# geometryxyz/mental-poker

Measured on AMD Instinct MI355X. Metric: shuffle proofs/sec (prove+verify), higher is better.
Workload: dtype u32 limbs (256-bit Montgomery: 9x29-bit lazy base field, 8x32 scalar field); 1 GPU; pairs: 52-card deck, m=2 n=26, stark curve, shuffle_and_remask + verify_shuffle; rccl_world=1, fixed_base_window_bits=21, unit_counted=prove+verify pairs, streams=1, aggregate_keys=1, transcript_lanes=1, prover_streams=1, pipeline_depth=0, validated_once=False, full=False

## Files before the change

mental-poker_amd/csrc/engine_core.hpp:

```cpp
#pragma once
#include "engine_base.hpp"
#include "kernels_bucket.hpp"
#include "kernels_canonical.hpp"
#include "kernels_sigma.hpp"
#include "kernels_open.hpp"
#include "kernels_deal.hpp"
#include "kernels_sample.hpp"
#include "kernels_screen.hpp"
#include "serialize_host.hpp"
#include "setup_host.hpp"

namespace mp {

static const uint32_t FCHUNK = 8;
static const uint32_t VCHUNK = 64;
static const uint32_t NORM_CHUNK = 64;
static const uint32_t BUCKET_MIN = 2048;
static const uint32_t BUCKET_MIN_SMALL_BATCH = 512;

struct PhaseDev {
  DevBuf<Term> recode, tables, fterms, vterms, cterms, cterms2, cterms0;
  DevBuf<Job> fjobs, vjobs, cjobs, cjobs2, cjobs0;
  DevBuf<BJob> bjobs;
  DevBuf<Term> bterms;
  DevBuf<BTermPos> bpos;
  DevBuf<Job> wcjobs;
  DevBuf<Term> wcterms;
  DevBuf<BJob> wjobs;
  uint32_t vsplit = 1, n_wc = 0, n_w = 0;
  uint32_t n_b = 0, n_bterms = 0, b_dig_bytes = 0, b_kpad_max = 0, b_bits = 8;
  uint32_t n_recode = 0, n_tables = 0, n_f = 0, n_v = 0, n_c = 0, n_c2 = 0, n_c0 = 0, n_tslots = 0, n_dslots = 0;
  std::vector<std::pair<uint32_t, uint32_t>> normalize;
  void upload(const Phase& ph, rt::Stream s) {
    recode.upload(ph.recode, s);
    tables.upload(ph.tables, s);
    fterms.upload(ph.fterms, s);
    vterms.upload(ph.vterms, s);
    cterms.upload(ph.cterms, s);
    fjobs.upload(ph.fjobs, s);
    vjobs.upload(ph.vjobs, s);
    cjobs.upload(ph.cjobs, s);
    cterms2.upload(ph.cterms2, s);
    cjobs2.upload(ph.cjobs2, s);
    n_c2 = (uint32_t)ph.cjobs2.size();
    cterms0.upload(ph.cterms0, s);
    cjobs0.upload(ph.cjobs0, s);
    n_c0 = (uint32_t)ph.cjobs0.size();
    wcjobs.upload(ph.wcjobs, s);
    wcterms.upload(ph.wcterms, s);
    wjobs.upload(ph.wjobs, s);
    vsplit = ph.vsplit;
    n_wc = (uint32_t)ph.wcjobs.size();
    n_w = (uint32_t)ph.wjobs.size();
    bjobs.upload(ph.bjobs, s);
    bterms.upload(ph.bterms, s);
    bpos.upload(ph.bpos, s);
    n_b = (uint32_t)ph.bjobs.size();
    n_bterms = (uint32_t)ph.bterms.size();
    b_dig_bytes = ph.b_dig_bytes;
    b_kpad_max = ph.b_kpad_max;
    b_bits = ph.b_bits;
    n_recode = (uint32_t)ph.recode.size();
    n_tables = (uint32_t)ph.tables.size();
    n_f = (uint32_t)ph.fjobs.size();
    n_v = (uint32_t)ph.vjobs.size();
    n_c = (uint32_t)ph.cjobs.size();
    n_tslots = ph.n_tslots;
    n_dslots = ph.n_dslots;
// ... 262 lines not shown
    rt::stream_sync(s);
  }
  DevBuf<uint32_t> vflag;
  uint32_t* flag_word(bool vlane, rt::Stream s) {
    if (!vflag.n) vflag.alloc(2, s);
    rt::dzero(vflag.p + (vlane ? 1 : 0), 4, s);
    return vflag.p + (vlane ? 1 : 0);
  }
  bool read_flag(bool vlane) {
    uint32_t flag = 0;
    rt::d2h(&flag, vflag.p + (vlane ? 1 : 0), 4, ctx->stream);
    rt::stream_sync(ctx->stream);
    return flag != 0;
  }
  uint32_t nwin = 0;
  FbGeom fbg{8, 32, 255};
  uint32_t init_seed[8];
  DevBuf<uint8_t> io_a, io_b, io_c, io_d, io_e, io_f;
  DevBuf<int32_t> io_status;

  static bool wire_point_host(const uint8_t* p, Aff<C>& out) {
    alignas(8) uint8_t tmp[G_::PB];
    memcpy(tmp, p, G_::PB);
    return wire_to_aff<C>(tmp, out);
  }

  void build_plans(PlanSet* set, bool keyed) {
    rt::Stream s = ctx->stream;
    for (int k = 0; k < N_PLANS; ++k) {
      PlanSet& q = set[k];
      const PlanParams& pp = pprm[k];
      const uint32_t bmin = (bucket_min && k == 3) ? std::min(bucket_min, BUCKET_MIN_SMALL_BATCH) : bucket_min;
      const uint32_t pbits = bucket_bits_of(4 * N + 11 * m + 9);
      q.pplan = make_prove_plan(m, n, pp.fch, pp.vch, G_::PB, keyed, bmin, bk_windows(R::BITS, pbits), toom_cook && (k == 0 || k == 2 || k == 4), pp.vsp, pbits);
      q.vplan = make_verify_plan(m, n, pp.fch, pp.vch, G_::PB, keyed, bmin, bk_windows(R::BITS, pbits), pp.vsp, pbits);
      q.table_group = pp.grp;
      q.norm_chunk = pp.nch;
      for (int i = 0; i < 6; ++i) q.pph[i].upload(q.pplan.ph[i], s);
      q.vph.upload(q.vplan.ph, s);
      q.vmph.upload(q.vplan.mph, s);
      q.mjobs.upload(q.vplan.mjobs, s);
      q.mpairs.upload(q.vplan.mpairs, s);
      q.draws.upload(q.pplan.draws, s);
      q.lin.upload(q.pplan.lin, s);
      q.lin_src.upload(q.pplan.lin_src, s);
      q.lin_coef.upload(q.pplan.lin_coef, s);
      q.consts.upload(toom_constants(q.pplan.toom), s);
      q.pwire.upload(q.pplan.wire, s);
      q.vwire.upload(q.vplan.wire, s);
    }
  }
  void ensure_keyed() {
    if (psk_ready) return;
    build_plans(psk, true);
    const ProveLay& l = psk[0].pplan.lay;
    key_d_first = key_t_first = 0;
    for (int k = 0; k < N_PLANS; ++k)
      for (int i = 0; i < 6; ++i) {
        key_d_first = std::max(key_d_first, psk[k].pplan.ph[i].n_dslots);
        key_t_first = std::max(key_t_first, psk[k].pplan.ph[i].n_tslots);
      }
    std::vector<Term> rec, tab;
    for (uint32_t i = 0; i < N; ++i) rec.push_back(Term{l.rho + i, key_d_first + i});
    for (uint32_t w = 0; w < nwin; ++w) tab.push_back(Term{l.kw + w, key_t_first + w});
    key_recode.upload(rec, ctx->stream);
    key_tables.upload(tab, ctx->stream);
    psk_ready = true;
// ... 187 lines not shown
    if (!scratch) scratch = w.NS.p;
    if (parts & PH_TABLES) run_tables(ph, w, B, scratch);
    if (parts & PH_RECODE) run_recode(ph, w, B);
    if (parts & PH_MSM) run_msms(ph, w, B);
    if (parts & PH_NORM) run_normalize(ph, w, B, norm_only, norm_skip, scratch);
  }
#ifdef MP_EXP_QUAD_MAX
  uint32_t quad_max_lanes = MP_EXP_QUAD_MAX;
#else
  uint32_t quad_max_lanes = 65536;
#endif
  bool quad_ops(uint32_t B, uint32_t njobs) const {
    const uint64_t items = (uint64_t)B * njobs;
    if (items > 0xFFFFFFF0ull) return false;
    return group_lanes == 4 || (group_lanes == 0 && items * 4u <= quad_max_lanes);
  }
  static uint32_t quad_waves(uint32_t B, uint32_t njobs) { return (uint32_t)(((uint64_t)B * njobs + 15u) / 16u); }
  void run_combine(const CombineArgs& a, uint32_t B, uint32_t njobs) {
    if (quad_ops(B, njobs)) {
      CombineQuadArgs qa{a, B, njobs};
      MP_WAVE_RUN(k_combine_q, C, quad_waves(B, njobs), 0, qa);
    } else {
      MP_RUN(k_combine, C, B, njobs, a);
    }
  }
  void run_recode(PhaseDev& ph, Workspace& w, uint32_t B) {
    if (ph.n_recode) {
      RecodeArgs a{w.S.p, w.D.p, ph.recode.p, w.Bpad, nwin};
      MP_RUN(k_recode, C, B, ph.n_recode, a);
    }
  }
  void run_tables(PhaseDev& ph, Workspace& w, uint32_t B, uint32_t* scratch) {
    if (ph.n_tables) {
      TableArgs a{w.P.p, w.T.p, scratch, ph.tables.p, w.Bpad, ph.n_tables, cur_table_group};
      MP_RUN(k_table, C, B, (ph.n_tables + cur_table_group - 1) / cur_table_group, a);
    }
  }

  uint32_t bk_pass_eqs = 0;
  size_t bk_pass_bytes = 0;
  uint32_t bucket_slots() {
    if (!ctx->bk_slots) ctx->bk_slots = BK_WAVES_PER_CU * rt::cu_count();
    return ctx->bk_slots;
  }
  void run_bucket(Workspace& w, PhaseDev& ph, const uint32_t* S, uint32_t sstride, int16_t* D, size_t dstride, uint32_t count,
                  uint32_t link_stride, const char* too_large, const uint32_t* tile = nullptr, uint32_t tile_K = 0) {
    rt::Stream s = ctx->stream;
    const uint32_t c = ph.b_bits, bw = bk_windows(R::BITS, c);
    if ((uint64_t)count * ph.n_bterms >= ((uint64_t)1 << 32) || (uint64_t)count * ph.n_b * bw + 8ull * bucket_slots() >= ((uint64_t)1 << 32)) throw std::runtime_error(too_large);
    BRecodeArgs ra{S, D, ph.bterms.p, ph.bpos.p, sstride, bw, ph.n_bterms, dstride, c};
    MP_RUN(k_bucket_recode, C, count * ph.n_bterms, 1, ra);
    if (c >= bucket_split_bits) {
      const uint32_t NBK = bk_buckets(c), XW = XyzzWords<C>::N, gmax = bk_chunks(ph.b_kpad_max), units = bk_units(c);
      if (gmax > BK_CHUNKS_MAX) throw std::runtime_error("bucket method: more than 589 824 terms in one multi-scalar multiplication with windows of 12 bits or more");
      const size_t per_item = ((size_t)ph.b_kpad_max + (size_t)NBK * XW) * 4 + (size_t)gmax * bk_offs_row(c) * 2, per_eq = per_item * ph.n_b * bw;
      if (!bk_pass_eqs || bk_pass_bytes != per_eq) {
        size_t free_b = 0, total_b = 0;
        rt::mem_info(&free_b, &total_b);
        const size_t have = (w.bk_sorted.n + w.bk_park.n) * 4 + w.bk_offs.n * 2;
        const size_t budget = total_b ? std::min<size_t>((size_t)12 << 30, (free_b + have) / 4) : (size_t)1 << 30;
        bk_pass_eqs = (uint32_t)std::max<size_t>(1, std::min<size_t>(budget / per_eq, 0x7FFFFFFFu));
        bk_pass_bytes = per_eq;
      }
      const uint32_t pass = std::min(count, std::max(bk_pass_eqs, 1u));
      const size_t items_max = (size_t)pass * ph.n_b * bw;
      if (items_max * units >= ((uint64_t)1 << 32)) throw std::runtime_error(too_large);
      w.bk_sorted.alloc(items_max * ph.b_kpad_max, s, false);
      w.bk_offs.alloc(items_max * gmax * bk_offs_row(c), s, false);
// ... 2124 lines not shown
```

mental-poker_amd/csrc/field.hpp:

```cpp
#pragma once
#include <cstdint>

#include "curve_params.hpp"
#include "rt.hpp"

namespace mp {

template <class P>
struct Fe {
  uint32_t v[P::L29 ? P::NL29 : P::NW];
};

static constexpr uint32_t M29 = (1u << 29) - 1;

template <class P>
MP_HD void fe_cond_sub(uint32_t* r, const uint32_t* a, uint32_t hi) {
  constexpr int N = P::NW;
  uint32_t d[N];
  uint64_t br = 0;
#pragma unroll
  for (int i = 0; i < N; ++i) {
    uint64_t t = (uint64_t)a[i] - P::MOD[i] - br;
    d[i] = (uint32_t)t;
    br = (t >> 32) & 1;
// ... 425 lines not shown
    reduce_carry29<P>(s, r.v);
    return r;
  } else {
    return fe_sub<P>(fe_sub<P>(a, u), fe_dbl<P>(v));
  }
}
template <class P>
MP_HD Fe<P> fe_sub_dbl(const Fe<P>& a, const Fe<P>& v) {
  if constexpr (P::L29 && !P::DENSE29) {
    Fe<P> r;
    int32_t s[P::NL29];
#pragma unroll
    for (int i = 0; i < P::NL29; ++i) s[i] = (int32_t)a.v[i] - 2 * (int32_t)v.v[i] + 4 * P::SMOD29[i];
    reduce_carry29<P>(s, r.v);
    return r;
  } else {
    return fe_sub<P>(a, fe_dbl<P>(v));
  }
}
template <class P>
MP_HD Fe<P> fe_triple_add(const Fe<P>& a, const Fe<P>& b) {
  if constexpr (P::L29 && !P::DENSE29) {
    Fe<P> r;
    int32_t s[P::NL29];
#pragma unroll
    for (int i = 0; i < P::NL29; ++i) s[i] = 3 * (int32_t)a.v[i] + (int32_t)b.v[i];
    reduce_carry29<P>(s, r.v);
    return r;
  } else {
    return fe_add<P>(fe_add<P>(fe_dbl<P>(a), a), b);
  }
}
template <class P>
struct LazySub {
  static constexpr bool ON = P::L29 && !P::PM29 && !P::DENSE29 && P::NL29 == 9;
  static constexpr int32_t k(int i) { return 8 * P::SMOD29[i] + (i == 0 ? (1 << 29) : i == 8 ? -1 : (1 << 29) - 1); }
};
template <class P>
MP_HD Fe<P> fe_sub_lazy(const Fe<P>& a, const Fe<P>& b) {
  if constexpr (LazySub<P>::ON) {
    Fe<P> r;
#pragma unroll
    for (int i = 0; i < 9; ++i) r.v[i] = a.v[i] - b.v[i] + (uint32_t)LazySub<P>::k(i);
    return r;
  } else {
    return fe_sub<P>(a, b);
  }
}
template <class P>
MP_HD Fe<P> fe_sub_wide(const Fe<P>& a, const Fe<P>& b) {
  if constexpr (LazySub<P>::ON) {
    Fe<P> r;
    int32_t s[9];
#pragma unroll
    for (int i = 0; i < 9; ++i) s[i] = (int32_t)a.v[i] - (int32_t)b.v[i] + 4 * P::SMOD29[i];
    carry29<9>(s, r.v);
    return r;
  } else {
    return fe_sub<P>(a, b);
  }
}
template <class P>
MP_HD Fe<P> fe_neg_lazy(const Fe<P>& a) {
  if constexpr (LazySub<P>::ON) {
    Fe<P> r;
#pragma unroll
// ... 313 lines not shown
```

mental-poker_amd/csrc/kernels_msm.hpp:

```cpp
#pragma once
#include "curve.hpp"
#include "layout.hpp"

namespace mp {

template <class C>
struct Geo {
  static constexpr int OCC4 = C::FqP::NW > 8 ? 2 : 4;
  static constexpr int OCC3 = C::FqP::NW > 8 ? 2 : 3;
#ifdef MP_OCC_VAR
  static constexpr int OCC_VAR = MP_OCC_VAR;
#else
  static constexpr int OCC_VAR = OCC4;
#endif
  static constexpr int OCC_TABLE = C::FqP::NW > 8 ? 2 : (C::FqP::L29 ? 4 : 3);
  static constexpr uint32_t FW = C::FqP::NW;
  static constexpr uint32_t PW = 2 * FW;
  static constexpr uint32_t JW = 3 * FW;
  static constexpr uint32_t FB = 4 * FW;
  static constexpr uint32_t PB = 8 * FW;
};
template <int N>
MP_HD void ld_words(const uint32_t* p, uint32_t* v) {
  static_assert(N % 4 == 0, "elements are whole 16-byte vectors");
// ... 268 lines not shown
  const Term* list;
  uint32_t Bpad, nwin;
};
template <class C>
MP_HD void body_recode(const RecodeArgs& a, uint32_t b, uint32_t y) {
  typedef typename C::FrP R;
  const Term t = a.list[y];
  uint32_t k[9];
  fe_to_canonical<R>(ld_fe<R>(a.S + s_off(t.s, a.Bpad, b)), k);
  k[8] = 0;
  int carry = 0;
  for (uint32_t w = 0; w < a.nwin; ++w) {
    const uint32_t bit = w * VB_WINDOW_BITS;
    const uint32_t lo = k[bit >> 5] >> (bit & 31);
    const uint32_t hi = (bit & 31) > 27 ? k[(bit >> 5) + 1] << (32 - (bit & 31)) : 0u;
    int d = (int)((lo | hi) & 31u) + carry;
    carry = 0;
    if (d > 16) {
      d -= 32;
      carry = 1;
    }
    a.D[((size_t)t.b * a.nwin + w) * a.Bpad + b] = (int8_t)d;
  }
}
MP_KERNEL(k_recode, RecodeArgs, body_recode)

static const uint32_t TABLE_GROUP = 64;
struct TableArgs {
  const uint32_t* P;
  uint32_t* T;
  uint32_t* scratch;
  const Term* list;
  uint32_t Bpad, n_tables, group;
};
MP_HD uint32_t table_key(uint32_t e0, uint32_t t) { return (e0 == 2 ? 4u : 0u) + (t - e0 - 1); }
template <class C>
MP_HD void table_emit(const TableArgs& a, uint32_t b, uint32_t ts, uint32_t e0n, uint32_t t, Fe<typename C::FqP>& prod,
                      const Fe<typename C::FqP>& den) {
  typedef typename C::FqP F;
  st_fe_lazy<F>(a.scratch + f_off<C>(ts * 8 + table_key(e0n, t), a.Bpad, b), prod);
  if (!fe_is_zero(den)) prod = fe_mul<F>(prod, den);
}
template <class C>
MP_HD Aff<C> table_step(const TableArgs& a, uint32_t b, uint32_t ts, uint32_t e0, uint32_t t, Fe<typename C::FqP>& inv,
                        const Aff<C>& lo, const Aff<C>& hi, bool dbl) {
  typedef typename C::FqP F;
  const Fe<F> den = dbl ? fe_dbl<F>(lo.y) : fe_sub_wide<F>(hi.x, lo.x);
  Aff<C> out = aff_inf<C>();
  if (!fe_is_zero(den)) {
    const Fe<F> dinv = fe_mul<F>(inv, ld_fe<F>(a.scratch + f_off<C>(ts * 8 + table_key(e0, t), a.Bpad, b)));
    inv = fe_mul<F>(inv, den);
    Fe<F> num;
    if (dbl) {
      const Fe<F> xx = fe_sqr<F>(lo.x);
      num = C::A == 1 ? fe_triple_add<F>(xx, fe_one<F>()) : fe_add<F>(fe_dbl<F>(xx), xx);
    } else {
      num = fe_sub<F>(hi.y, lo.y);
    }
    const Fe<F> lam = fe_mul<F>(num, dinv);
    const Fe<F>& x2 = dbl ? lo.x : hi.x;
    out.x = fe_sub<F>(fe_sub<F>(fe_sqr<F>(lam), lo.x), x2);
    out.y = fe_sub<F>(fe_mul<F>(lam, fe_sub_lazy<F>(lo.x, out.x)), lo.y);
  }
  st_aff_lazy<C>(a.T + p_off<C>(ts * VB_ENTRIES + t - 1, a.Bpad, b), out);
  return out;
}
template <class C>
MP_HD void body_table(const TableArgs& a, uint32_t b, uint32_t y) {
  typedef typename C::FqP F;
  const uint32_t g0 = y * a.group;
  const uint32_t g1 = g0 + a.group < a.n_tables ? g0 + a.group : a.n_tables;
  Fe<F> prod = fe_one<F>();
  for (uint32_t g = g0; g < g1; ++g) {
    const Term t = a.list[g];
    const Aff<C> p1 = ld_aff<C>(a.P + p_off<C>(t.s, a.Bpad, b));
    st_aff<C>(a.T + p_off<C>(t.b * VB_ENTRIES, a.Bpad, b), p1);
    table_emit<C>(a, b, t.b, 1, 2, prod, fe_dbl<F>(p1.y));
  }
  bool desc = true;
#pragma unroll 1
  for (uint32_t e0 = 1; e0 < (uint32_t)VB_ENTRIES; e0 *= 2, desc = !desc) {
    Fe<F> inv = fe_inv<F>(prod);
    prod = fe_one<F>();
    const bool emit = 2 * e0 < (uint32_t)VB_ENTRIES;
    const uint32_t e0n = 2 * e0;
    for (uint32_t gi = 0; gi < g1 - g0; ++gi) {
      const uint32_t g = desc ? g1 - 1 - gi : g0 + gi;
      const uint32_t ts = a.list[g].b;
      const uint32_t* tb = a.T + p_off<C>(ts * VB_ENTRIES, a.Bpad, b);
      const size_t estride = (size_t)a.Bpad * Geo<C>::PW;
      if (e0 == 1) {
        const Aff<C> lo = ld_aff<C>(tb);
        const Aff<C> o2 = table_step<C>(a, b, ts, 1, 2, inv, lo, lo, true);
        table_emit<C>(a, b, ts, e0n, 4, prod, fe_dbl<F>(o2.y));
        table_emit<C>(a, b, ts, e0n, 3, prod, fe_sub<F>(o2.x, lo.x));
        continue;
      }
      const uint32_t h = e0 / 2;
// ... 9 lines not shown
          }
          const Aff<C> out = table_step<C>(a, b, ts, e0, t, inv, lo, hi, dbl);
          if (emit) {
            if (t < 2 * e0) table_emit<C>(a, b, ts, e0n, 2 * t + 1, prod, fe_sub<F>(prevx, out.x));
            table_emit<C>(a, b, ts, e0n, 2 * t, prod, fe_dbl<F>(out.y));
            prevx = out.x;
          }
        }
        if (emit)
          table_emit<C>(a, b, ts, e0n, 2 * e0 + 1, prod, fe_sub<F>(prevx, ld_fe<F>(tb + (size_t)(e0 - 1) * estride)));
      } else {
        Aff<C> lo = ld_aff<C>(tb + (size_t)(h - 1) * estride), hi = lo;
        Fe<F> prevx = lo.x;
        if (emit) prevx = ld_fe<F>(tb + (size_t)(e0 - 1) * estride);
#pragma unroll 1
        for (uint32_t t = e0 + 1; t <= 2 * e0; ++t) {
          const bool dbl = (t & 1u) == 0;
          if (!dbl) {
            if (t != e0 + 1) lo = hi;
            hi = ld_aff<C>(tb + (size_t)((t + 1) / 2 - 1) * estride);
          } else {
            lo = hi;
          }
          const Aff<C> out = table_step<C>(a, b, ts, e0, t, inv, lo, hi, dbl);
          if (emit) {
            table_emit<C>(a, b, ts, e0n, 2 * t - 1, prod, fe_sub<F>(out.x, prevx));
            table_emit<C>(a, b, ts, e0n, 2 * t, prod, fe_dbl<F>(out.y));
            prevx = out.x;
          }
        }
      }
    }
  }
}
MP_KERNEL_OCC(k_table, TableArgs, body_table, Geo<C>::OCC_TABLE)

struct VarArgs {
  const int8_t* D;
  const uint32_t* T;
  uint32_t* J;
  const Job* jobs;
  const Term* terms;
  uint32_t Bpad, nwin;
  uint32_t split;
};
template <class C>
MP_HD void body_var_msm(const VarArgs& a, uint32_t b, uint32_t y) {
  const uint32_t jidx = a.split > 1 ? y / a.split : y, r = y - jidx * a.split;
  const Job job = a.jobs[jidx];
  const int w_top = a.split > 1 ? (int)vsplit_lo(r + 1, a.split, a.nwin) - 1 : (int)a.nwin - 1;
  const int w_low = a.split > 1 ? (int)vsplit_lo(r, a.split, a.nwin) : 0;
  Xyzz<C> acc = xyzz_inf<C>();
#pragma unroll 1
  for (int w = w_top; w >= w_low; --w) {
    if (w != w_top) {
#pragma unroll 1
      for (int q = 0; q < VB_WINDOW_BITS; ++q) xyzz_dbl_ip<C>(acc);
    }
#pragma unroll 1
    for (uint32_t t = 0; t < job.count; ++t) {
      const Term term = a.terms[job.begin + t];
      const int d = a.D[((size_t)term.s * a.nwin + w) * a.Bpad + b];
      if (d != 0) {
        const uint32_t e = (uint32_t)(d < 0 ? -d : d) - 1;
        const Aff<C> q = ld_aff<C>(a.T + p_off<C>(term.b * VB_ENTRIES + e, a.Bpad, b));
        xyzz_madd_signed_ip<C>(acc, q, d < 0);
// ... 264 lines not shown
```

mental-poker_amd/csrc/layout.hpp:

```cpp
#pragma once
#include <algorithm>
#include <cstdint>
#include <map>
#include <stdexcept>
#include <vector>

#include "rt.hpp"

namespace mp {

struct Job {
  uint32_t out;
  uint32_t begin;
  uint32_t count;
};
struct Term {
  uint32_t s;
  uint32_t b;
};
struct BJob {
  uint32_t out;
  uint32_t win_first;
  uint32_t begin;
  uint32_t count;
  uint32_t kpad;
  uint32_t dig_off;
};
struct BTermPos {
  uint32_t pos;
  uint32_t kpad;
};
static const uint32_t AFF_FLAG = 0x80000000u;
static const uint32_t NEG_FLAG = 0x40000000u;
static const uint32_t SLOT_MASK = 0x3FFFFFFFu;
static const uint32_t NO_SLOT = 0xFFFFFFFFu;

struct FixedBases {
  uint32_t n;
  MP_HD uint32_t ck(uint32_t j) const { return j; }
  MP_HD uint32_t H() const { return n; }
  MP_HD uint32_t G() const { return n + 1; }
  MP_HD uint32_t pk() const { return n + 2; }
  MP_HD uint32_t gen() const { return n + 3; }
  MP_HD uint32_t gsum() const { return n + 4; }
  MP_HD uint32_t count() const { return n + 5; }
};

static const int VB_WINDOW_BITS = 5;
static const int VB_ENTRIES = 16;
static const uint32_t KEY_WINDOWS = 52;
static inline int vb_windows(int scalar_bits) { return (scalar_bits + 1 + VB_WINDOW_BITS - 1) / VB_WINDOW_BITS; }
MP_HD uint32_t vsplit_lo(uint32_t r, uint32_t k, uint32_t nwin) { return r * nwin / k; }
static const uint32_t VSPLIT_MAX = 16;

struct Phase {
  std::vector<Term> recode;
  std::vector<Term> tables;
  std::vector<Job> fjobs, vjobs, cjobs, cjobs2;
  std::vector<Term> fterms, vterms, cterms, cterms2;
  std::vector<Job> cjobs0;
  std::vector<Term> cterms0;
  std::vector<std::pair<uint32_t, uint32_t>> normalize;
  uint32_t n_dslots = 0, n_tslots = 0;
  uint32_t vsplit = 1;
  std::vector<Job> wcjobs;
  std::vector<Term> wcterms;
  std::vector<BJob> wjobs;
  std::vector<BJob> bjobs;
  std::vector<Term> bterms;
  std::vector<BTermPos> bpos;
  uint32_t b_dig_bytes = 0;
  uint32_t b_kpad_max = 0;
  uint32_t b_bits = 8;
};

static const size_t COMBINE_TREE_MIN = 12;
static const size_t BUCKET_TERMS_MAX = 589824;
class PhaseBuilder {
 public:
  PhaseBuilder(Phase& ph, uint32_t& next_partial, uint32_t fchunk, uint32_t vchunk, uint32_t bucket_min = 0, uint32_t bwin = 0,
               uint32_t vsplit = 1, uint32_t bbits = 8)
      : ph_(ph), next_partial_(next_partial), fchunk_(fchunk), vchunk_(vchunk), bucket_min_(bucket_min), bwin_(bwin),
        vsplit_(vsplit < 1 ? 1 : (vsplit > VSPLIT_MAX ? VSPLIT_MAX : vsplit)) {
    ph_.vsplit = vsplit_;
    ph_.b_bits = bbits;
  }
  void begin(uint32_t out_slot) {
    out_ = out_slot;
    f_.clear();
    v_.clear();
    a_.clear();
  }
  void fixed(uint32_t sslot, uint32_t base) { f_.push_back(Term{sslot, base}); }
  void var(uint32_t sslot, uint32_t pslot) { v_.push_back(Term{sslot, pslot}); }
  void addend(uint32_t pslot, bool negate = false) { a_.push_back(AFF_FLAG | (negate ? NEG_FLAG : 0u) | pslot); }
  void addend_j(uint32_t jslot, bool negate = false) { a_.push_back((negate ? NEG_FLAG : 0u) | jslot); }
  uint32_t new_partial() { return next_partial_++; }
  void end(bool late = false) {
    const size_t MAXP = 128;
    size_t fchunk_ = this->fchunk_, vchunk_ = this->vchunk_;
    const bool bucket = bucket_min_ && v_.size() >= bucket_min_ && v_.size() <= BUCKET_TERMS_MAX;
    if (!bucket)
      for (Term& t : v_) t = Term{dslot(t.s), tslot(t.b)};
    if ((f_.size() + fchunk_ - 1) / fchunk_ > MAXP) fchunk_ = (f_.size() + MAXP - 1) / MAXP;
    if ((v_.size() + vchunk_ - 1) / vchunk_ > MAXP) vchunk_ = (v_.size() + MAXP - 1) / MAXP;
    size_t nf = (f_.size() + fchunk_ - 1) / fchunk_, nv = bucket ? 1 : (v_.size() + vchunk_ - 1) / vchunk_;
    const bool wsplit = !bucket && vsplit_ > 1 && nv > 0;
    size_t pieces = nf + (wsplit ? 1 : nv) + a_.size();
    if (pieces == 0) throw std::logic_error("empty msm");
    bool direct = pieces == 1 && a_.empty();
    std::vector<uint32_t> parts;
    for (size_t c = 0; c < nf; ++c) {
      uint32_t out = direct ? out_ : next_partial_++;
      size_t b = c * fchunk_, e = std::min(f_.size(), b + fchunk_);
      ph_.fjobs.push_back(Job{out, (uint32_t)ph_.fterms.size(), (uint32_t)(e - b)});
      ph_.fterms.insert(ph_.fterms.end(), f_.begin() + b, f_.begin() + e);
      parts.push_back(out);
    }
    if (bucket) {
      const uint32_t out = direct ? out_ : next_partial_++;
      const uint32_t kpad = (uint32_t)((v_.size() + 63) / 64 * 64);
      BJob bj{out, next_partial_, (uint32_t)ph_.bterms.size(), (uint32_t)v_.size(), kpad, ph_.b_dig_bytes};
      next_partial_ += bwin_;
      for (size_t i = 0; i < v_.size(); ++i) ph_.bpos.push_back(BTermPos{ph_.b_dig_bytes + (uint32_t)i, kpad});
      ph_.bterms.insert(ph_.bterms.end(), v_.begin(), v_.end());
      ph_.b_dig_bytes += bwin_ * kpad;
      ph_.b_kpad_max = std::max(ph_.b_kpad_max, kpad);
      ph_.bjobs.push_back(bj);
      parts.push_back(out);
    }
    if (wsplit) {
      std::vector<uint32_t> first(nv);
      for (size_t c = 0; c < nv; ++c) {
        first[c] = next_partial_;
        next_partial_ += vsplit_;
        size_t b = c * vchunk_, e = std::min(v_.size(), b + vchunk_);
// ... 39 lines not shown
      }
      cj.push_back(Job{out_, (uint32_t)ct.size(), (uint32_t)parts.size()});
      for (uint32_t p : parts) ct.push_back(Term{p, 0});
    }
  }
  void normalize(uint32_t first, uint32_t count) {
    if (count) ph_.normalize.push_back({first, count});
  }

 private:
  uint32_t dslot(uint32_t sslot) {
    auto it = dmap_.find(sslot);
    if (it != dmap_.end()) return it->second;
    uint32_t d = ph_.n_dslots++;
    dmap_[sslot] = d;
    ph_.recode.push_back(Term{sslot, d});
    return d;
  }
  uint32_t tslot(uint32_t pslot) {
    auto it = tmap_.find(pslot);
    if (it != tmap_.end()) return it->second;
    uint32_t t = ph_.n_tslots++;
    tmap_[pslot] = t;
    ph_.tables.push_back(Term{pslot, t});
    return t;
  }
  Phase& ph_;
  uint32_t& next_partial_;
  uint32_t fchunk_, vchunk_, bucket_min_, bwin_, vsplit_;
  uint32_t out_ = 0;
  std::vector<Term> f_, v_;
  std::vector<uint32_t> a_;
  std::map<uint32_t, uint32_t> dmap_, tmap_;
};

struct ProveLay {
  uint32_t m, n, N;
  uint32_t rho, a, b, tmp, r, s, sb, hs, dz, t, bp, zB, zs, za0, zbm, zr0, zsm, zt, zd;
  uint32_t svbp, svd, svrd, svdelta, svs1, svsx, svv1, svv2;
  uint32_t mea0, mer0, meb, mes, metau;
  uint32_t tsp, tsm;
  uint32_t x, y, z, hx, hy, zx, svx, mx;
  uint32_t zabar, zbbar, zrbar, zsbar, ztbar, svat, svbt, svrt, svst, meabar, merbar, mebbar, mesbar, metaubar;
  uint32_t nS, tmp_len;
  uint32_t deck, shuf, cA, cB, cb, hB, zcA0, zcBm, zcD, svcd, svcdelta, svcDelta, mecA0, mecB, meE;
  uint32_t tDp, tDm;
  uint32_t pk, kw;
  uint32_t nP;
  uint32_t n_draws;
  uint32_t toom;
};

struct VerifyLay {
  uint32_t m, n, N;
  uint32_t zabar, zbbar, zrbar, zsbar, ztbar, svat, svbt, svrt, svst, meabar, merbar, mebbar, mesbar, metaubar;
  uint32_t x, y, z, hx, hy, zx, svx, mx, one, tmp, coef;
  uint32_t nS, tmp_len, n_coef;
  uint32_t deck, shuf, cA, cB, cb, hB, zcA0, zcBm, zcD, svcd, svcdelta, svcDelta, mecA0, mecB, meE;
  uint32_t pk;
  uint32_t nP;
  uint32_t chk_first, n_chk;
  uint32_t mr, mvar, mfix, chk_merged;
};

struct ProofElem {
  uint32_t is_point;
// ... 75 lines not shown
  R(l.svd, n); R(l.svrd, 1);
  if (n > 2) R(l.svdelta + 1, n - 2);
  R(l.svs1, 1); R(l.svsx, 1);
  R(l.mea0, n); R(l.mer0, 1); R(l.meb, 2 * m); R(l.mes, 2 * m); R(l.metau, 2 * m);
  return d;
}

struct LinJob {
  uint32_t dst, begin, count;
};

struct ToomPlan {
  uint32_t E = 0;
  uint32_t sv_first = 0;
  uint32_t cv_first = 0;
  uint32_t pp_first = 0;
  uint32_t w_first = 0;
  uint32_t n_consts = 0, w_const_first = 0;
  static uint32_t pair_x(uint32_t p) { return p == 0 ? 1u : (p + 1) / 2 + 1; }
  static bool pair_rev(uint32_t p) { return p != 0 && (p & 1u) == 0; }
  int32_t x_of(uint32_t e) const {
    const int32_t x = (int32_t)pair_x((e - 2) / 2);
    return (e & 1u) ? -x : x;
  }
  bool rev_of(uint32_t e) const { return pair_rev((e - 2) / 2); }
};
static const uint32_t TOOM_MAX_M = 16;
struct ProvePlan {
  ProveLay lay;
  std::vector<LinJob> lin;
  std::vector<uint32_t> lin_src;
  std::vector<uint32_t> lin_coef;
  ToomPlan toom;
  Phase ph[6];
  uint32_t nJ;
  uint32_t jkey = NO_SLOT;
  std::vector<uint32_t> draws;
  std::vector<ProofElem> wire;
};

struct KLeaf {
  std::vector<uint32_t> a, c;
  std::map<uint32_t, int> contrib;
};
typedef std::vector<std::vector<uint32_t>> KPoly;
static inline std::vector<uint32_t> k_union(const std::vector<uint32_t>& x, const std::vector<uint32_t>& y) {
  std::vector<uint32_t> r(x);
  r.insert(r.end(), y.begin(), y.end());
  std::sort(r.begin(), r.end());
  return r;
}
static inline void k_append(std::vector<KLeaf>& dst, const std::vector<KLeaf>& src, uint32_t shift, int sign) {
  for (const KLeaf& s : src) {
    KLeaf t;
    t.a = s.a;
    t.c = s.c;
    for (auto& kv : s.contrib) t.contrib[kv.first + shift] = sign * kv.second;
    dst.push_back(t);
  }
}
static inline std::vector<KLeaf> k_mul(const KPoly& A, const KPoly& C) {
  std::vector<KLeaf> out;
  if (A.empty() || C.empty()) return out;
  if (A.size() == 1 || C.size() == 1) {
    for (uint32_t j = 0; j < A.size(); ++j)
      for (uint32_t t = 0; t < C.size(); ++t) {
// ... 17 lines not shown
  KPoly As(A0), Cs(C0);
  for (size_t i = 0; i < A1.size(); ++i) As[i] = k_union(A0[i], A1[i]);
  for (size_t i = 0; i < C1.size(); ++i) Cs[i] = k_union(C0[i], C1[i]);
  const std::vector<KLeaf> P0 = k_mul(A0, C0), P2 = k_mul(A1, C1), P1 = k_mul(As, Cs);
  k_append(out, P0, 0, 1);
  k_append(out, P2, 2 * h, 1);
  k_append(out, P1, h, 1);
  k_append(out, P0, h, -1);
  k_append(out, P2, h, -1);
  return out;
}
static inline std::vector<KLeaf> k_merge(const std::vector<KLeaf>& in) {
  std::map<std::pair<std::vector<uint32_t>, std::vector<uint32_t>>, std::map<uint32_t, int>> acc;
  std::vector<std::pair<std::vector<uint32_t>, std::vector<uint32_t>>> order;
  for (const KLeaf& lf : in) {
    auto key = std::make_pair(lf.a, lf.c);
    if (!acc.count(key)) order.push_back(key);
    for (auto& kv : lf.contrib) acc[key][kv.first] += kv.second;
  }
  std::vector<KLeaf> out;
  for (auto& key : order) {
    KLeaf lf;
    lf.a = key.first;
    lf.c = key.second;
    for (auto& kv : acc[key])
      if (kv.second != 0) lf.contrib[kv.first] = kv.second;
    if (!lf.contrib.empty()) out.push_back(lf);
  }
  return out;
}

static inline ProvePlan make_prove_plan(uint32_t m, uint32_t n, uint32_t fchunk, uint32_t vchunk, uint32_t point_bytes = 64,
                                        bool keyed = false, uint32_t bucket_min = 0, uint32_t bwin = 0, bool toom_cook = true,
                                        uint32_t vsplit = 1, uint32_t bbits = 8) {
  ProvePlan pl;
  pl.lay = make_prove_lay(m, n);
  pl.lay.toom = m == 2 ? 1u : 0u;
  const bool toomk = toom_cook && m >= 3 && m <= TOOM_MAX_M;
  const bool karatsuba = m >= 3 && !toomk;
  if (toomk) {
    ToomPlan& T = pl.toom;
    T.E = 2 * m;
    T.sv_first = pl.lay.nS;
    pl.lay.nS += (T.E - 2) * n;
    T.w_first = pl.lay.nS;
    pl.lay.nS += T.E * T.E;
    T.cv_first = pl.lay.nP;
    pl.lay.nP += (T.E - 2) * 2 * n;
    T.pp_first = pl.lay.nP;
    pl.lay.nP += 2 * T.E;
    T.w_const_first = T.E * (m + 1);
    T.n_consts = T.w_const_first + T.E * T.E;
    for (uint32_t e = 2; e < T.E; ++e) {
      pl.lin.push_back(LinJob{T.sv_first + (e - 2) * n, (uint32_t)pl.lin_src.size(), m + 1});
      for (uint32_t j = 0; j <= m; ++j) {
        pl.lin_src.push_back(j == 0 ? pl.lay.mea0 : pl.lay.b + (j - 1) * n);
        pl.lin_coef.push_back(e * (m + 1) + j);
      }
    }
  }
  std::vector<KLeaf> leaves;
  std::map<std::vector<uint32_t>, uint32_t> svec, cvec;
  uint32_t kP0 = pl.lay.nP;
  if (karatsuba) {
    KPoly A, Cc;
    for (uint32_t j = 0; j <= m; ++j) A.push_back({j});
    for (uint32_t t = 0; t < m; ++t) Cc.push_back({m - t - 1});
    leaves = k_merge(k_mul(A, Cc));
    for (const KLeaf& lf : leaves) {
      for (auto& kv : lf.contrib)
// ... 7 lines not shown
          for (uint32_t j : lf.a) pl.lin_src.push_back(j == 0 ? pl.lay.mea0 : pl.lay.b + (j - 1) * n);
          pl.lay.nS += n;
        }
      }
      if (!cvec.count(lf.c)) {
        if (lf.c.size() == 1) {
          cvec[lf.c] = pl.lay.shuf + 2 * lf.c[0] * n;
        } else {
          cvec[lf.c] = pl.lay.nP;
          pl.lay.nP += 2 * n;
        }
      }
    }
  }
  const ProveLay& l = pl.lay;
  FixedBases fb{n};
  uint32_t next_partial = l.nP;
  if (keyed) {
    pl.jkey = next_partial;
    next_partial += 2 * m;
  }
  auto commit = [&](PhaseBuilder& B, uint32_t out, uint32_t vec, uint32_t len, uint32_t rslot) {
    B.begin(out);
    for (uint32_t j = 0; j < len; ++j) B.fixed(vec + j, fb.ck(j));
    B.fixed(rslot, fb.H());
    B.end();
  };
  {
    PhaseBuilder B(pl.ph[0], next_partial, fchunk, vchunk, bucket_min, bwin, vsplit, bbits);
    for (uint32_t k = 0; k < m; ++k) commit(B, l.cA + k, l.a + k * n, n, l.r + k);
    B.normalize(l.shuf, 2 * l.N);
    B.normalize(l.cA, m);
  }
  if (pl.lay.toom) {
    PhaseBuilder B(pl.ph[4], next_partial, fchunk, vchunk, bucket_min, bwin, vsplit, bbits);
    for (uint32_t t = 0; t < n; ++t)
      for (uint32_t c = 0; c < 2; ++c) {
        B.begin(l.tDp + 2 * t + c);
        B.addend(l.shuf + 2 * t + c);
        B.addend(l.shuf + 2 * (n + t) + c);
        B.end();
        B.begin(l.tDm + 2 * t + c);
        B.addend(l.shuf + 2 * (n + t) + c);
        B.addend(l.shuf + 2 * t + c, true);
        B.end();
      }
    B.normalize(l.tDp, 4 * n);
  }
  if (karatsuba && l.nP > kP0) {
    PhaseBuilder B(pl.ph[4], next_partial, fchunk, vchunk, bucket_min, bwin, vsplit, bbits);
    for (auto& kv : cvec) {
      if (kv.first.size() == 1) continue;
      for (uint32_t t = 0; t < n; ++t)
        for (uint32_t c = 0; c < 2; ++c) {
          B.begin(kv.second + 2 * t + c);
          for (uint32_t r : kv.first) B.addend(l.shuf + 2 * (r * n + t) + c);
          B.end();
        }
    }
    B.normalize(kP0, l.nP - kP0);
  }
  {
    PhaseBuilder B(pl.ph[1], next_partial, fchunk, vchunk, bucket_min, bwin, vsplit, bbits);
    for (uint32_t k = 0; k < m; ++k) commit(B, l.cB + k, l.b + k * n, n, l.s + k);
    commit(B, l.mecA0, l.mea0, n, l.mer0);
    for (uint32_t k = 0; k < 2 * m; ++k) commit(B, l.mecB + k, l.meb + k, 1, l.mes + k);
    const bool toom = pl.lay.toom != 0;
    if (toom) {
      for (uint32_t c = 0; c < 2; ++c) {
        const uint32_t v0 = B.new_partial(), vinf = B.new_partial(), v1 = B.new_partial(), vm1 = B.new_partial();
        B.begin(v0);
        for (uint32_t t = 0; t < n; ++t) B.var(l.mea0 + t, l.shuf + 2 * (n + t) + c);
        B.end();
        B.begin(vinf);
        for (uint32_t t = 0; t < n; ++t) B.var(l.b + n + t, l.shuf + 2 * t + c);
        B.end();
        B.begin(v1);
        for (uint32_t t = 0; t < n; ++t) B.var(l.tsp + t, l.tDp + 2 * t + c);
        B.end();
        B.begin(vm1);
        for (uint32_t t = 0; t < n; ++t) B.var(l.tsm + t, l.tDm + 2 * t + c);
        B.end();
        for (uint32_t k = 0; k < 4; ++k) {
          B.begin(l.meE + 2 * k + c);
          if (c == 0) {
            B.fixed(l.metau + k, fb.G());
          } else {
            B.fixed(l.meb + k, fb.gen());
            if (keyed) B.addend_j(pl.jkey + k); else B.fixed(l.metau + k, fb.pk());
          }
          if (k == 0) B.addend_j(v0);
          if (k == 3) B.addend_j(vinf);
          if (k == 1) { B.addend_j(v1); B.addend_j(vm1, true); B.addend_j(vinf, true); }
          if (k == 2) { B.addend_j(v1); B.addend_j(vm1); B.addend_j(v0, true); }
          B.end(true);
        }
      }
    } else if (toomk) {
      const ToomPlan& T = pl.toom;
      for (uint32_t e = 0; e < T.E; ++e)
        for (uint32_t c = 0; c < 2; ++c) {
          const uint32_t sv = e == 0 ? l.mea0 : (e == 1 ? l.b + (m - 1) * n : T.sv_first + (e - 2) * n);
          const uint32_t cv = e == 0 ? l.shuf + 2 * (m - 1) * n : (e == 1 ? l.shuf : T.cv_first + (e - 2) * 2 * n);
          B.begin(T.pp_first + 2 * e + c);
          for (uint32_t t = 0; t < n; ++t) B.var(sv + t, cv + 2 * t + c);
          B.end();
        }
      B.normalize(T.pp_first, 2 * T.E);
    } else if (karatsuba) {
      for (uint32_t c = 0; c < 2; ++c) {
        std::vector<uint32_t> part(leaves.size());
        for (size_t i = 0; i < leaves.size(); ++i) {
          part[i] = B.new_partial();
          const uint32_t sv = svec[leaves[i].a], cv = cvec[leaves[i].c];
// ... 337 lines not shown
```

Baseline: 733,700 proofs/s.

## Derive Toom sum/difference point tables from base tables via batched affine addition

For m=2 Toom proving, the sum and difference points (P+Q, Q-P) and their precomputed multiple tables are no longer built as separate normalized partials in phase 4. They are now computed directly inside the table kernel from the existing base-point tables. One batched Montgomery inversion per group shares a denominator between the plus and minus entries, with an exact XYZZ fallback for degenerate pairs. A fused fe_sub_sub is also added for the x-coordinate. This removes one phase and its normalization, at the cost of more table-kernel work and a larger group size when pairs are present.

```diff
diff --git a/mental-poker_amd/csrc/engine_core.hpp b/mental-poker_amd/csrc/engine_core.hpp
--- a/mental-poker_amd/csrc/engine_core.hpp
+++ b/mental-poker_amd/csrc/engine_core.hpp
@@ -20,6 +20,8 @@
 
 struct PhaseDev {
   DevBuf<Term> recode, tables, fterms, vterms, cterms, cterms2, cterms0;
+  DevBuf<TablePair> pairs;
+  uint32_t n_pairs = 0;
   DevBuf<Job> fjobs, vjobs, cjobs, cjobs2, cjobs0;
   DevBuf<BJob> bjobs;
   DevBuf<Term> bterms;
@@ -34,6 +36,8 @@
   void upload(const Phase& ph, rt::Stream s) {
     recode.upload(ph.recode, s);
     tables.upload(ph.tables, s);
+    pairs.upload(ph.pairs, s);
+    n_pairs = (uint32_t)ph.pairs.size();
     fterms.upload(ph.fterms, s);
     vterms.upload(ph.vterms, s);
     cterms.upload(ph.cterms, s);
@@ -362,7 +366,8 @@
       const PlanParams& pp = pprm[k];
       const uint32_t bmin = (bucket_min && k == 3) ? std::min(bucket_min, BUCKET_MIN_SMALL_BATCH) : bucket_min;
       const uint32_t pbits = bucket_bits_of(4 * N + 11 * m + 9);
-      q.pplan = make_prove_plan(m, n, pp.fch, pp.vch, G_::PB, keyed, bmin, bk_windows(R::BITS, pbits), toom_cook && (k == 0 || k == 2 || k == 4), pp.vsp, pbits);
+      q.pplan = make_prove_plan(m, n, pp.fch, pp.vch, G_::PB, keyed, bmin, bk_windows(R::BITS, pbits), toom_cook && (k == 0 || k == 2 || k == 4), pp.vsp, pbits,
+                                Cofactor<C>::ONE);
       q.vplan = make_verify_plan(m, n, pp.fch, pp.vch, G_::PB, keyed, bmin, bk_windows(R::BITS, pbits), pp.vsp, pbits);
       q.table_group = pp.grp;
       q.norm_chunk = pp.nch;
@@ -616,8 +621,9 @@
   }
   void run_tables(PhaseDev& ph, Workspace& w, uint32_t B, uint32_t* scratch) {
     if (ph.n_tables) {
-      TableArgs a{w.P.p, w.T.p, scratch, ph.tables.p, w.Bpad, ph.n_tables, cur_table_group};
-      MP_RUN(k_table, C, B, (ph.n_tables + cur_table_group - 1) / cur_table_group, a);
+      const uint32_t group = ph.n_pairs ? std::min((cur_table_group + 1u) & ~1u, TABLE_GROUP) : cur_table_group;
+      TableArgs a{w.P.p, w.T.p, scratch, ph.tables.p, w.Bpad, ph.n_tables, group, ph.pairs.p, ph.n_pairs};
+      MP_RUN(k_table, C, B, (ph.n_tables + group - 1) / group, a);
     }
   }
 
diff --git a/mental-poker_amd/csrc/field.hpp b/mental-poker_amd/csrc/field.hpp
--- a/mental-poker_amd/csrc/field.hpp
+++ b/mental-poker_amd/csrc/field.hpp
@@ -481,6 +481,19 @@
   }
 }
 template <class P>
+MP_HD Fe<P> fe_sub_sub(const Fe<P>& a, const Fe<P>& u, const Fe<P>& v) {
+  if constexpr (P::L29 && !P::DENSE29) {
+    Fe<P> r;
+    int32_t s[P::NL29];
+#pragma unroll
+    for (int i = 0; i < P::NL29; ++i) s[i] = (int32_t)a.v[i] - (int32_t)u.v[i] - (int32_t)v.v[i] + 8 * P::SMOD29[i];
+    reduce_carry29<P>(s, r.v);
+    return r;
+  } else {
+    return fe_sub<P>(fe_sub<P>(a, u), v);
+  }
+}
+template <class P>
 struct LazySub {
   static constexpr bool ON = P::L29 && !P::PM29 && !P::DENSE29 && P::NL29 == 9;
   static constexpr int32_t k(int i) { return 8 * P::SMOD29[i] + (i == 0 ? (1 << 29) : i == 8 ? -1 : (1 << 29) - 1); }
diff --git a/mental-poker_amd/csrc/kernels_msm.hpp b/mental-poker_amd/csrc/kernels_msm.hpp
--- a/mental-poker_amd/csrc/kernels_msm.hpp
+++ b/mental-poker_amd/csrc/kernels_msm.hpp
@@ -324,6 +324,8 @@
   uint32_t* scratch;
   const Term* list;
   uint32_t Bpad, n_tables, group;
+  const TablePair* pairs;
+  uint32_t n_pairs;
 };
 MP_HD uint32_t table_key(uint32_t e0, uint32_t t) { return (e0 == 2 ? 4u : 0u) + (t - e0 - 1); }
 template <class C>
@@ -351,11 +353,98 @@
     }
     const Fe<F> lam = fe_mul<F>(num, dinv);
     const Fe<F>& x2 = dbl ? lo.x : hi.x;
-    out.x = fe_sub<F>(fe_sub<F>(fe_sqr<F>(lam), lo.x), x2);
+    out.x = fe_sub_sub<F>(fe_sqr<F>(lam), lo.x, x2);
     out.y = fe_sub<F>(fe_mul<F>(lam, fe_sub_lazy<F>(lo.x, out.x)), lo.y);
   }
   st_aff_lazy<C>(a.T + p_off<C>(ts * VB_ENTRIES + t - 1, a.Bpad, b), out);
   return out;
+}
+template <class C>
+MP_HD bool table_pair_generic(const Aff<C>& p1, const Aff<C>& q1) {
+  typedef typename C::FqP F;
+  return !aff_is_inf<C>(p1) && !aff_is_inf<C>(q1) && !fe_is_zero(fe_sub<F>(q1.x, p1.x));
+}
+MP_HD uint32_t table_pair_key(const TablePair& pr, uint32_t k) { return (k <= 8 ? pr.tdp : pr.tdm) * 8 + ((k - 1) & 7u); }
+template <class C>
+MP_HD Aff<C> xyzz_to_aff(const Xyzz<C>& p) {
+  typedef typename C::FqP F;
+  if (fe_is_zero(p.ZZ)) return aff_inf<C>();
+  const Fe<F> zi3 = fe_inv<F>(p.ZZZ), zi = fe_mul<F>(p.ZZ, zi3);
+  Aff<C> r;
+  r.x = fe_mul<F>(p.X, fe_sqr<F>(zi));
+  r.y = fe_mul<F>(p.Y, zi3);
+  return r;
+}
+template <class C>
+MP_HD_NOINLINE void table_pair_exact(const TableArgs& a, uint32_t b, const TablePair& pr) {
+  const size_t estride = (size_t)a.Bpad * Geo<C>::PW;
+  const uint32_t* tp = a.T + p_off<C>(pr.tp * VB_ENTRIES, a.Bpad, b);
+  const uint32_t* tq = a.T + p_off<C>(pr.tq * VB_ENTRIES, a.Bpad, b);
+#pragma unroll 1
+  for (uint32_t k = 0; k < 2u * VB_ENTRIES; ++k) {
+    const uint32_t e = k >> 1;
+    const bool minus = (k & 1u) != 0;
+    Xyzz<C> acc = xyzz_inf<C>();
+    xyzz_madd_ip<C>(acc, ld_aff<C>(tq + e * estride));
+    xyzz_madd_signed_ip<C>(acc, ld_aff<C>(tp + e * estride), minus);
+    st_aff_lazy<C>(a.T + p_off<C>((minus ? pr.tdm : pr.tdp) * VB_ENTRIES + e, a.Bpad, b), xyzz_to_aff<C>(acc));
+  }
+}
+template <class C>
+MP_HD void table_pairs(const TableArgs& a, uint32_t b, uint32_t p0, uint32_t p1) {
+  typedef typename C::FqP F;
+  const size_t estride = (size_t)a.Bpad * Geo<C>::PW;
+  Fe<F> prod = fe_one<F>();
+  uint32_t smask = 0;
+  for (uint32_t p = p0; p < p1; ++p) {
+    const TablePair pr = a.pairs[p];
+    const uint32_t* tp = a.T + p_off<C>(pr.tp * VB_ENTRIES, a.Bpad, b);
+    const uint32_t* tq = a.T + p_off<C>(pr.tq * VB_ENTRIES, a.Bpad, b);
+    if (!table_pair_generic<C>(ld_aff<C>(tp), ld_aff<C>(tq))) {
+      smask |= 1u << (p - p0);
+      continue;
+    }
+#pragma unroll 1
+    for (uint32_t k0 = 0; k0 < (uint32_t)VB_ENTRIES; k0 += 4) {
+      Fe<F> den[4];
+#pragma unroll
+      for (uint32_t j = 0; j < 4; ++j)
+        den[j] = fe_sub<F>(ld_fe<F>(tq + (k0 + j) * estride), ld_fe<F>(tp + (k0 + j) * estride));
+#pragma unroll
+      for (uint32_t j = 0; j < 4; ++j) {
+        st_fe_lazy<F>(a.scratch + f_off<C>(table_pair_key(pr, k0 + j + 1), a.Bpad, b), prod);
+        prod = fe_mul<F>(prod, den[j]);
+      }
+    }
+  }
+  const uint32_t all = p1 - p0 >= 32 ? 0xFFFFFFFFu : (1u << (p1 - p0)) - 1u;
+  if (smask != all) {
+    Fe<F> inv = fe_inv<F>(prod);
+    for (uint32_t p = p1; p-- > p0;) {
+      if ((smask >> (p - p0)) & 1u) continue;
+      const TablePair pr = a.pairs[p];
+      const uint32_t* tp = a.T + p_off<C>(pr.tp * VB_ENTRIES, a.Bpad, b);
+      const uint32_t* tq = a.T + p_off<C>(pr.tq * VB_ENTRIES, a.Bpad, b);
+#pragma unroll 1
+      for (uint32_t k = VB_ENTRIES; k >= 1; --k) {
+        const Aff<C> P = ld_aff<C>(tp + (k - 1) * estride), Q = ld_aff<C>(tq + (k - 1) * estride);
+        const Fe<F> dinv = fe_mul<F>(inv, ld_fe<F>(a.scratch + f_off<C>(table_pair_key(pr, k), a.Bpad, b)));
+        inv = fe_mul<F>(inv, fe_sub<F>(Q.x, P.x));
+        const Fe<F> lp = fe_mul<F>(fe_sub<F>(Q.y, P.y), dinv), lm = fe_mul<F>(fe_add<F>(Q.y, P.y), dinv);
+        Aff<C> dp, dm;
+        dp.x = fe_sub_sub<F>(fe_sqr<F>(lp), P.x, Q.x);
+        dp.y = fe_sub<F>(fe_mul<F>(lp, fe_sub_lazy<F>(P.x, dp.x)), P.y);
+        dm.x = fe_sub_sub<F>(fe_sqr<F>(lm), P.x, Q.x);
+        dm.y = fe_sub<F>(fe_mul<F>(lm, fe_sub_lazy<F>(Q.x, dm.x)), Q.y);
+        st_aff_lazy<C>(a.T + p_off<C>(pr.tdp * VB_ENTRIES + k - 1, a.Bpad, b), dp);
+        st_aff_lazy<C>(a.T + p_off<C>(pr.tdm * VB_ENTRIES + k - 1, a.Bpad, b), dm);
+      }
+    }
+  }
+  if (smask) {
+    for (uint32_t p = p0; p < p1; ++p)
+      if ((smask >> (p - p0)) & 1u) table_pair_exact<C>(a, b, a.pairs[p]);
+  }
 }
 template <class C>
 MP_HD void body_table(const TableArgs& a, uint32_t b, uint32_t y) {
@@ -431,6 +520,8 @@
       }
     }
   }
+  const uint32_t p0 = g0 / 2, p1 = g1 / 2 < a.n_pairs ? g1 / 2 : a.n_pairs;
+  if (p0 < p1) table_pairs<C>(a, b, p0, p1);
 }
 MP_KERNEL_OCC(k_table, TableArgs, body_table, Geo<C>::OCC_TABLE)
 
diff --git a/mental-poker_amd/csrc/layout.hpp b/mental-poker_amd/csrc/layout.hpp
--- a/mental-poker_amd/csrc/layout.hpp
+++ b/mental-poker_amd/csrc/layout.hpp
@@ -53,9 +53,14 @@
 MP_HD uint32_t vsplit_lo(uint32_t r, uint32_t k, uint32_t nwin) { return r * nwin / k; }
 static const uint32_t VSPLIT_MAX = 16;
 
+struct TablePair {
+  uint32_t tp, tq, tdp, tdm;
+};
+
 struct Phase {
   std::vector<Term> recode;
   std::vector<Term> tables;
+  std::vector<TablePair> pairs;
   std::vector<Job> fjobs, vjobs, cjobs, cjobs2;
   std::vector<Term> fterms, vterms, cterms, cterms2;
   std::vector<Job> cjobs0;
@@ -74,6 +79,7 @@
   uint32_t b_bits = 8;
 };
 
+static const uint32_t DERIVED_FLAG = 0x80000000u;
 static const size_t COMBINE_TREE_MIN = 12;
 static const size_t BUCKET_TERMS_MAX = 589824;
 class PhaseBuilder {
@@ -93,6 +99,21 @@
   }
   void fixed(uint32_t sslot, uint32_t base) { f_.push_back(Term{sslot, base}); }
   void var(uint32_t sslot, uint32_t pslot) { v_.push_back(Term{sslot, pslot}); }
+  void var_derived(uint32_t sslot, uint32_t tslot) { v_.push_back(Term{sslot, DERIVED_FLAG | tslot}); }
+  TablePair derived_pair(uint32_t pslot_p, uint32_t pslot_q) {
+    auto it = pmap_.find({pslot_p, pslot_q});
+    if (it != pmap_.end()) return ph_.pairs[it->second];
+    if (ph_.tables.size() != 2 * ph_.pairs.size() || tmap_.count(pslot_p) || tmap_.count(pslot_q) || pslot_p == pslot_q)
+      throw std::logic_error("derived table pairs must lead the table list");
+    TablePair pr;
+    pr.tp = tslot(pslot_p);
+    pr.tq = tslot(pslot_q);
+    pr.tdp = ph_.n_tslots++;
+    pr.tdm = ph_.n_tslots++;
+    pmap_[{pslot_p, pslot_q}] = (uint32_t)ph_.pairs.size();
+    ph_.pairs.push_back(pr);
+    return pr;
+  }
   void addend(uint32_t pslot, bool negate = false) { a_.push_back(AFF_FLAG | (negate ? NEG_FLAG : 0u) | pslot); }
   void addend_j(uint32_t jslot, bool negate = false) { a_.push_back((negate ? NEG_FLAG : 0u) | jslot); }
   uint32_t new_partial() { return next_partial_++; }
@@ -100,8 +121,10 @@
     const size_t MAXP = 128;
     size_t fchunk_ = this->fchunk_, vchunk_ = this->vchunk_;
     const bool bucket = bucket_min_ && v_.size() >= bucket_min_ && v_.size() <= BUCKET_TERMS_MAX;
+    for (const Term& t : v_)
+      if (bucket && (t.b & DERIVED_FLAG)) throw std::logic_error("a derived table cannot feed a bucket job");
     if (!bucket)
-      for (Term& t : v_) t = Term{dslot(t.s), tslot(t.b)};
+      for (Term& t : v_) t = Term{dslot(t.s), (t.b & DERIVED_FLAG) ? (t.b & ~DERIVED_FLAG) : tslot(t.b)};
     if ((f_.size() + fchunk_ - 1) / fchunk_ > MAXP) fchunk_ = (f_.size() + MAXP - 1) / MAXP;
     if ((v_.size() + vchunk_ - 1) / vchunk_ > MAXP) vchunk_ = (v_.size() + MAXP - 1) / MAXP;
     size_t nf = (f_.size() + fchunk_ - 1) / fchunk_, nv = bucket ? 1 : (v_.size() + vchunk_ - 1) / vchunk_;
@@ -207,6 +230,7 @@
   std::vector<Term> f_, v_;
   std::vector<uint32_t> a_;
   std::map<uint32_t, uint32_t> dmap_, tmap_;
+  std::map<std::pair<uint32_t, uint32_t>, uint32_t> pmap_;
 };
 
 struct ProveLay {
@@ -348,6 +372,7 @@
   std::vector<uint32_t> lin_src;
   std::vector<uint32_t> lin_coef;
   ToomPlan toom;
+  bool pair_tables = false;
   Phase ph[6];
   uint32_t nJ;
   uint32_t jkey = NO_SLOT;
@@ -431,10 +456,11 @@
 
 static inline ProvePlan make_prove_plan(uint32_t m, uint32_t n, uint32_t fchunk, uint32_t vchunk, uint32_t point_bytes = 64,
                                         bool keyed = false, uint32_t bucket_min = 0, uint32_t bwin = 0, bool toom_cook = true,
-                                        uint32_t vsplit = 1, uint32_t bbits = 8) {
+                                        uint32_t vsplit = 1, uint32_t bbits = 8, bool pair_tables = true) {
   ProvePlan pl;
   pl.lay = make_prove_lay(m, n);
   pl.lay.toom = m == 2 ? 1u : 0u;
+  pl.pair_tables = pair_tables && m == 2 && !(bucket_min && n >= bucket_min && n <= BUCKET_TERMS_MAX);
   const bool toomk = toom_cook && m >= 3 && m <= TOOM_MAX_M;
   const bool karatsuba = m >= 3 && !toomk;
   if (toomk) {
@@ -508,7 +534,7 @@
     B.normalize(l.shuf, 2 * l.N);
     B.normalize(l.cA, m);
   }
-  if (pl.lay.toom) {
+  if (pl.lay.toom && !pl.pair_tables) {
     PhaseBuilder B(pl.ph[4], next_partial, fchunk, vchunk, bucket_min, bwin, vsplit, bbits);
     for (uint32_t t = 0; t < n; ++t)
       for (uint32_t c = 0; c < 2; ++c) {
@@ -543,6 +569,10 @@
     for (uint32_t k = 0; k < 2 * m; ++k) commit(B, l.mecB + k, l.meb + k, 1, l.mes + k);
     const bool toom = pl.lay.toom != 0;
     if (toom) {
+      std::vector<TablePair> dpair(2 * n);
+      if (pl.pair_tables)
+        for (uint32_t t = 0; t < n; ++t)
+          for (uint32_t c = 0; c < 2; ++c) dpair[2 * t + c] = B.derived_pair(l.shuf + 2 * t + c, l.shuf + 2 * (n + t) + c);
       for (uint32_t c = 0; c < 2; ++c) {
         const uint32_t v0 = B.new_partial(), vinf = B.new_partial(), v1 = B.new_partial(), vm1 = B.new_partial();
         B.begin(v0);
@@ -552,10 +582,12 @@
         for (uint32_t t = 0; t < n; ++t) B.var(l.b + n + t, l.shuf + 2 * t + c);
         B.end();
         B.begin(v1);
-        for (uint32_t t = 0; t < n; ++t) B.var(l.tsp + t, l.tDp + 2 * t + c);
+        for (uint32_t t = 0; t < n; ++t)
+          if (pl.pair_tables) B.var_derived(l.tsp + t, dpair[2 * t + c].tdp); else B.var(l.tsp + t, l.tDp + 2 * t + c);
         B.end();
         B.begin(vm1);
-        for (uint32_t t = 0; t < n; ++t) B.var(l.tsm + t, l.tDm + 2 * t + c);
+        for (uint32_t t = 0; t < n; ++t)
+          if (pl.pair_tables) B.var_derived(l.tsm + t, dpair[2 * t + c].tdm); else B.var(l.tsm + t, l.tDm + 2 * t + c);
         B.end();
         for (uint32_t k = 0; k < 4; ++k) {
           B.begin(l.meE + 2 * k + c);
```

Measured after the change: 737,100 proofs/s (median of 6 runs). Within noise of the previous version (+0.5%).
